# pathwaycom/pathway

Hardware: AMD Instinct MI355X
Metric: events/sec (whole node) on WordCount stream + p50 RAG query latency at fixed QPS (higher is better)
Workload: dtype int64/string-dict; 1 GPU; model=wordcount: stream -> groupby(word).count -> output deltas, global_batch=4000000, seq_len=1, parallelism=dp1 (shard exchange: RCCL all-to-all), vocab=50000, ingest=bytes, emitted_delta_rows=126750000, dict_misses=0

## Files before the change

pathway_amd/ops/__init__.py:

```python

from __future__ import annotations

import contextlib
import ctypes
import os
from typing import Sequence

import torch

_THIS = os.path.dirname(os.path.abspath(__file__))
_LIB_PATH = os.path.join(_THIS, "libpwhip.so")

_lib = None
_load_error: Exception | None = None


def _try_load():
    global _lib, _load_error
    if _lib is not None:
        return _lib
    try:
        if not os.path.exists(_LIB_PATH):
            from pathway_amd.ops import build as _build

# ... 1301 lines not shown
    vals = torch.empty((nq, k), dtype=torch.float32, device=scores.device)
    idx = torch.empty((nq, k), dtype=torch.int64, device=scores.device)
    if nq == 0:
        return vals, idx
    rc = lib.pw_topk(
        ctypes.c_void_p(scores.contiguous().data_ptr()),
        ctypes.c_int64(nq),
        ctypes.c_int64(m),
        ctypes.c_int(k),
        ctypes.c_void_p(vals.data_ptr()),
        ctypes.c_void_p(idx.data_ptr()),
        _stream_ptr(),
    )
    if rc != 0:
        raise RuntimeError(f"pw_topk failed: hip error {rc}")
    return vals, idx


BM25_TILE = 4096


def bm25_score(
    offsets: torch.Tensor,
    pidx: torch.Tensor,
    ptf: torch.Tensor,
    norm: torch.Tensor,
    q_off: torch.Tensor,
    q_term: torch.Tensor,
    q_idf: torch.Tensor,
    k1: float,
    pad_to: int = 1,
) -> torch.Tensor:
    n = norm.shape[0]
    nq = q_off.shape[0] - 1
    assert offsets.dtype == torch.int64 and pidx.dtype == torch.int32
    assert ptf.dtype == torch.float32 and norm.dtype == torch.float32
    assert q_off.dtype == torch.int32 and q_term.dtype == torch.int32
    assert q_idf.dtype == torch.float32
    assert pidx.shape == ptf.shape and q_term.shape == q_idf.shape
    assert nq >= 0 and offsets.shape[0] >= 1
    k1p1 = float(k1) + 1.0
    n_pad = -(-n // pad_to) * pad_to
    if not norm.is_cuda:
        scores = torch.zeros((nq, n_pad), dtype=torch.float32)
        k1p1_t = torch.tensor(k1p1, dtype=torch.float32)
        qo = q_off.tolist()
        for q in range(nq):
            row = scores[q]
            for t in range(qo[q], qo[q + 1]):
                term = int(q_term[t])
                s, e = int(offsets[term]), int(offsets[term + 1])
                d = pidx[s:e].long()
                tf = ptf[s:e]
                row.index_add_(0, d, q_idf[t] * (tf * k1p1_t) / (tf + norm[d]))
        return scores
    lib = require_lib()
    assert BM25_TILE == lib.pw_bm25_tile(), "BM25_TILE out of step with the kernel"
    scores = torch.empty((nq, n_pad), dtype=torch.float32, device=norm.device)
    if n_pad > n:
        scores[:, n:] = 0.0
    rc = lib.pw_bm25_score(
        ctypes.c_void_p(offsets.contiguous().data_ptr()),
        ctypes.c_void_p(pidx.contiguous().data_ptr()),
        ctypes.c_void_p(ptf.contiguous().data_ptr()),
        ctypes.c_void_p(norm.contiguous().data_ptr()),
        ctypes.c_int64(n),
        ctypes.c_void_p(q_off.contiguous().data_ptr()),
        ctypes.c_void_p(q_term.contiguous().data_ptr()),
        ctypes.c_void_p(q_idf.contiguous().data_ptr()),
        ctypes.c_int64(nq),
        ctypes.c_float(k1p1),
        ctypes.c_void_p(scores.data_ptr()),
        ctypes.c_int64(n_pad),
        _stream_ptr(),
    )
    if rc != 0:
        raise RuntimeError(f"pw_bm25_score failed: hip error {rc}")
    return scores


def merge_consolidate_gpu(
    a_words: Sequence[torch.Tensor],
    a_accs: Sequence[torch.Tensor],
    b_words: Sequence[torch.Tensor],
    b_accs: Sequence[torch.Tensor],
    compare_words: int | None = None,
) -> tuple[list[torch.Tensor], list[torch.Tensor], torch.Tensor]:
    lib = require_lib()
    m = a_words[0].shape[0]
    n = b_words[0].shape[0]
    nw = len(a_words)
    nwc = compare_words or nw
    nacc = len(a_accs)
    assert len(b_accs) == nacc and 1 <= nacc <= 8 and 1 <= nwc <= nw <= 4
    device = a_words[0].device
    total_diag = m + n
    nthreads = max(1, (total_diag + 7) // 8)
    counts = torch.empty(nthreads, dtype=torch.int32, device=device)
    wA = [t.contiguous() for t in a_words]
    wB = [t.contiguous() for t in b_words]
    aA = [t.contiguous() for t in a_accs]
    aB = [t.contiguous() for t in b_accs]
    rc = lib.pw_merge_consolidate_count(
        _ptr_arr(wA),
        _ptr_arr(aA),
        _ptr_arr(wB),
        _ptr_arr(aB),
        ctypes.c_int(nw),
        ctypes.c_int(nwc),
        ctypes.c_int(nacc),
        ctypes.c_int64(m),
        ctypes.c_int64(n),
        ctypes.c_void_p(counts.data_ptr()),
        ctypes.c_int64(nthreads),
        _stream_ptr(),
    )
    if rc != 0:
        raise RuntimeError(f"pw_merge_consolidate_count failed: {rc}")
    csum = torch.cumsum(counts.to(torch.int64), 0)
    total = int(csum[-1].item())
    bases = torch.zeros(nthreads, dtype=torch.int64, device=device)
    bases[1:] = csum[:-1]
    out_words = [
        torch.empty(total, dtype=torch.int64, device=device)
        for _ in range(nw)
    ]
    out_accs = [
        torch.empty(total, dtype=torch.int64, device=device)
        for _ in range(nacc)
    ]
    rep = torch.empty(total, dtype=torch.int64, device=device)
    rc = lib.pw_merge_consolidate_emit(
        _ptr_arr(wA),
        _ptr_arr(aA),
        _ptr_arr(wB),
        _ptr_arr(aB),
        ctypes.c_int(nw),
        ctypes.c_int(nwc),
        ctypes.c_int(nacc),
        ctypes.c_int64(m),
        ctypes.c_int64(n),
        ctypes.c_void_p(bases.data_ptr()),
        ctypes.c_int64(nthreads),
        _ptr_arr(out_words),
        _ptr_arr(out_accs),
        ctypes.c_void_p(rep.data_ptr()),
        _stream_ptr(),
    )
    if rc != 0:
        raise RuntimeError(f"pw_merge_consolidate_emit failed: {rc}")
    return out_words, out_accs, rep


def group_update_gpu(
    a_words: Sequence[torch.Tensor],
    a_accs: Sequence[torch.Tensor],
    b_words: Sequence[torch.Tensor],
    b_accs: Sequence[torch.Tensor],
    out_slots: Sequence[int],
):
    lib = require_lib()
    m = a_words[0].shape[0]
    n = b_words[0].shape[0]
    nacc = len(a_accs)
    assert len(a_words) == 2 and len(b_words) == 2
    assert len(b_accs) == nacc and 1 <= nacc <= 8
    slots = sorted(set(int(s) for s in out_slots))
    assert all(0 <= s < nacc for s in slots)
    mask = 0
    for s in slots:
        mask |= 1 << s
    device = b_words[0].device
    nthreads = max(1, (m + n + 7) // 8)
    counts = torch.empty(nthreads * 4, dtype=torch.int32, device=device)
    bases = torch.empty(nthreads * 3, dtype=torch.int64, device=device)
    totals = torch.empty(3, dtype=torch.int64, device=device)
    wA = [t.contiguous() for t in a_words]
    wB = [t.contiguous() for t in b_words]
    aA = [t.contiguous() for t in a_accs]
    aB = [t.contiguous() for t in b_accs]
    for t in wA + wB + aA + aB:
        assert t.dtype == torch.int64
    rc = lib.pw_group_update_count(
        _ptr_arr(wA),
        _ptr_arr(aA),
        _ptr_arr(wB),
        _ptr_arr(aB),
        ctypes.c_int(nacc),
        ctypes.c_uint(mask),
        ctypes.c_int64(m),
        ctypes.c_int64(n),
        ctypes.c_void_p(counts.data_ptr()),
        ctypes.c_void_p(bases.data_ptr()),
        ctypes.c_void_p(totals.data_ptr()),
        ctypes.c_int64(nthreads),
        _stream_ptr(),
    )
    if rc != 0:
        raise RuntimeError(f"pw_group_update_count failed: {rc}")
    n_keep, n_ret, n_ins = totals.tolist()
    n_out = n_ret + n_ins

    def i64(k):
        return torch.empty(k, dtype=torch.int64, device=device)

    out_words = [i64(n_keep) for _ in range(2)]
    out_accs = [i64(n_keep) for _ in range(nacc)]
    rep = i64(n_keep)
    keys = torch.empty((n_out, 2), dtype=torch.int64, device=device)
    diffs = i64(n_out)
    vals = {s: i64(n_out) for s in slots}
    src = i64(n_out)
    varr = (ctypes.c_void_p * 8)(
        *[ctypes.c_void_p(vals[s].data_ptr() if s in vals else 0) for s in range(8)]
    )
    rc = lib.pw_group_update_emit(
        _ptr_arr(wA),
        _ptr_arr(aA),
        _ptr_arr(wB),
        _ptr_arr(aB),
        ctypes.c_int(nacc),
        ctypes.c_uint(mask),
        ctypes.c_int64(m),
        ctypes.c_int64(n),
        ctypes.c_void_p(bases.data_ptr()),
        ctypes.c_int64(n_ret),
        ctypes.c_int64(nthreads),
        _ptr_arr(out_words),
        _ptr_arr(out_accs),
        ctypes.c_void_p(rep.data_ptr()),
        ctypes.c_void_p(keys.data_ptr()),
        ctypes.c_void_p(diffs.data_ptr()),
        varr,
        ctypes.c_void_p(src.data_ptr()),
        _stream_ptr(),
    )
    if rc != 0:
        raise RuntimeError(f"pw_group_update_emit failed: {rc}")
    return out_words, out_accs, rep, keys, diffs, [vals[s] for s in slots], src


def radix_sort64_gpu(keys: torch.Tensor) -> tuple[torch.Tensor, torch.Tensor]:
    lib = require_lib()
    n = keys.shape[0]
    device = keys.device
    perm = torch.arange(n, dtype=torch.int64, device=device)
    if n <= 1:
        return keys.clone(), perm
    nblocks = max(1, min(1024, (n + (64 * 64) - 1) // (64 * 64)))
    chunk = (n + nblocks * 64 - 1) // (nblocks * 64)
    ka = torch.empty(n, dtype=torch.int64, device=device)
    kb = torch.empty(n, dtype=torch.int64, device=device)
    pa = perm
    pb = torch.empty(n, dtype=torch.int64, device=device)
    rc = lib.pw_radix_flip(
        ctypes.c_void_p(keys.contiguous().data_ptr()),
        ctypes.c_void_p(ka.data_ptr()),
        ctypes.c_int64(n),
        _stream_ptr(),
    )
    if rc != 0:
        raise RuntimeError(f"pw_radix_flip failed: {rc}")
    counts = torch.empty(256 * nblocks, dtype=torch.int32, device=device)
    for p in range(8):
        shift = p * 8
        rc = lib.pw_radix_count(
            ctypes.c_void_p(ka.data_ptr()),
            ctypes.c_int64(n),
            ctypes.c_int(shift),
            ctypes.c_int64(nblocks),
            ctypes.c_int64(chunk),
            ctypes.c_void_p(counts.data_ptr()),
            _stream_ptr(),
        )
        if rc != 0:
            raise RuntimeError(f"pw_radix_count failed: {rc}")
        csum = torch.cumsum(counts.to(torch.int64), 0)
        bases = torch.zeros_like(csum)
        bases[1:] = csum[:-1]
        rc = lib.pw_radix_scatter(
            ctypes.c_void_p(ka.data_ptr()),
            ctypes.c_void_p(pa.data_ptr()),
            ctypes.c_int64(n),
            ctypes.c_int(shift),
            ctypes.c_int64(nblocks),
            ctypes.c_int64(chunk),
            ctypes.c_void_p(bases.data_ptr()),
            ctypes.c_void_p(kb.data_ptr()),
            ctypes.c_void_p(pb.data_ptr()),
            _stream_ptr(),
        )
        if rc != 0:
            raise RuntimeError(f"pw_radix_scatter failed: {rc}")
        ka, kb = kb, ka
        pa, pb = pb, pa
    out = torch.empty(n, dtype=torch.int64, device=device)
    rc = lib.pw_radix_unflip(
        ctypes.c_void_p(ka.data_ptr()),
        ctypes.c_void_p(out.data_ptr()),
        ctypes.c_int64(n),
        _stream_ptr(),
    )
    if rc != 0:
        raise RuntimeError(f"pw_radix_unflip failed: {rc}")
    return out, pa


def scan_positions_gpu(buf: torch.Tensor, target: int) -> torch.Tensor:
    lib = require_lib()
    n = buf.shape[0]
    device = buf.device
    nblocks = max(1, min(2048, (n + 4095) // 4096))
    counts = torch.empty(nblocks, dtype=torch.int64, device=device)
    rc = lib.pw_scan_positions(
        ctypes.c_void_p(buf.contiguous().data_ptr()),
        ctypes.c_int64(n),
        ctypes.c_int(int(target)),
        ctypes.c_void_p(counts.data_ptr()),
        ctypes.c_int64(nblocks),
        _stream_ptr(),
    )
    if rc != 0:
        raise RuntimeError(f"pw_scan_positions failed: {rc}")
    csum = torch.cumsum(counts, 0)
    total = int(csum[-1].item())
    bases = torch.zeros(nblocks, dtype=torch.int64, device=device)
    bases[1:] = csum[:-1]
    out = torch.empty(total, dtype=torch.int64, device=device)
    rc = lib.pw_scan_emit(
        ctypes.c_void_p(buf.contiguous().data_ptr()),
        ctypes.c_int64(n),
        ctypes.c_int(int(target)),
        ctypes.c_void_p(bases.data_ptr()),
        ctypes.c_int64(nblocks),
        ctypes.c_void_p(out.data_ptr()),
        _stream_ptr(),
    )
    if rc != 0:
        raise RuntimeError(f"pw_scan_emit failed: {rc}")
    return out


def sort_repair_gpu(
    k0_sorted: torch.Tensor,
    k1_sorted: torch.Tensor,
    perm: torch.Tensor,
    passes: int = 4,
) -> None:
    lib = require_lib()
    n = k0_sorted.shape[0]
    if n < 2:
        return
    rc = lib.pw_sort_repair(
        ctypes.c_void_p(k0_sorted.data_ptr()),
        ctypes.c_void_p(k1_sorted.data_ptr()),
        ctypes.c_void_p(perm.data_ptr()),
        ctypes.c_int64(n),
        ctypes.c_int(int(passes)),
        _stream_ptr(),
    )
    if rc != 0:
        raise RuntimeError(f"pw_sort_repair failed: hip error {rc}")


def gather_cols_gpu(idx: torch.Tensor, cols: list) -> list:
    lib = require_lib()
    m = idx.shape[0]
    outs: list = [None] * len(cols)
    fused_pos: list[int] = []
    for i, c in enumerate(cols):
        if c.dim() == 1 and c.element_size() == 8 and c.is_contiguous():
            fused_pos.append(i)
        else:
            outs[i] = c[idx] if c.dim() > 1 else c.index_select(0, idx)
    idx = idx.contiguous()
    for start in range(0, len(fused_pos), 8):
        group = fused_pos[start : start + 8]
        srcs = (ctypes.c_void_p * len(group))()
        dsts = (ctypes.c_void_p * len(group))()
        for k, i in enumerate(group):
# ... 210 lines not shown
```

pathway_amd/ops/csrc/hip/pw_kernels.hip:

```cpp
#include <hip/hip_runtime.h>
#include <stdint.h>
#include <stdio.h>

#include <cstring>
#include <rocprim/rocprim.hpp>

#include "../xxhash_common.h"

#define PW_BLOCK 256
#define PW_MAX_GRID 2048

static inline int pw_grid(int64_t n) {
  int64_t g = (n + PW_BLOCK - 1) / PW_BLOCK;
  if (g > PW_MAX_GRID) g = PW_MAX_GRID;
  if (g < 1) g = 1;
  return (int)g;
}


struct WordPtrs {
  const uint64_t* p[20];
};

template <int W>
// ... 942 lines not shown
__device__ int64_t mc_merge_path(McWords A, int64_t m, McWords B, int64_t n,
                                 int64_t d, int nwc) {
  int64_t lo = d > n ? d - n : 0;
  int64_t hi = d < m ? d : m;
  while (lo < hi) {
    int64_t mid = (lo + hi) >> 1;
    if (mc_le(A, mid, B, d - mid - 1, nwc))
      lo = mid + 1;
    else
      hi = mid;
  }
  return lo;
}

#define PW_MC_CHUNK 8

template <bool WRITE>
__device__ void mc_walk(McWords A, McAcc accA, McWords B, McAcc accB,
                        int nw, int nwc, int nacc, int64_t m, int64_t n,
                        int64_t d0, int64_t d1, int* count_out,
                        int64_t base, McWordsMut O, McAccMut accO,
                        int64_t* rep) {
  int64_t ai = mc_merge_path(A, m, B, n, d0, nwc);
  int64_t bi = d0 - ai;
  int64_t d = d0;
  if (d < d1 && bi < n && ai > 0 &&
      !(ai < m && mc_le(A, ai, B, bi, nwc))) {
    if (mc_eq(A, ai - 1, B, bi, nwc)) {
      ++bi;
      ++d;
    }
  }
  int cnt = 0;
  int64_t w = base;
  while (d < d1) {
    bool take_a = (bi >= n) || (ai < m && mc_le(A, ai, B, bi, nwc));
    if (take_a) {
      bool matched = (bi < n) && mc_eq(A, ai, B, bi, nwc);
      long long wsum = accA.p[0][ai] + (matched ? accB.p[0][bi] : 0ll);
      if (wsum != 0) {
        if (WRITE) {
          for (int k = 0; k < nw; ++k) O.p[k][w] = A.p[k][ai];
          for (int c = 0; c < nacc; ++c)
            accO.p[c][w] =
                accA.p[c][ai] + (matched ? accB.p[c][bi] : 0ll);
          rep[w] = ai;
          ++w;
        }
        ++cnt;
      }
      ++ai;
      ++d;
      if (matched) {
        ++bi;
        ++d;
      }
    } else {
      long long wsum = accB.p[0][bi];
      if (wsum != 0) {
        if (WRITE) {
          for (int k = 0; k < nw; ++k) O.p[k][w] = B.p[k][bi];
          for (int c = 0; c < nacc; ++c) accO.p[c][w] = accB.p[c][bi];
          rep[w] = m + bi;
          ++w;
        }
        ++cnt;
      }
      ++bi;
      ++d;
    }
  }
  if (!WRITE) *count_out = cnt;
}

__global__ void k_mc_count(McWords A, McAcc accA, McWords B, McAcc accB,
                           int nw, int nwc, int nacc, int64_t m, int64_t n,
                           int* thread_counts, int64_t nthreads) {
  int64_t t = (int64_t)blockIdx.x * blockDim.x + threadIdx.x;
  if (t >= nthreads) return;
  int64_t total = m + n;
  int64_t d0 = t * PW_MC_CHUNK;
  int64_t d1 = min(d0 + PW_MC_CHUNK, total);
  McAccMut dummy{};
  McWordsMut wdummy{};
  mc_walk<false>(A, accA, B, accB, nw, nwc, nacc, m, n, d0, d1,
                 &thread_counts[t], 0, wdummy, dummy, nullptr);
}

__global__ void k_mc_emit(McWords A, McAcc accA, McWords B, McAcc accB,
                          int nw, int nwc, int nacc, int64_t m, int64_t n,
                          const int64_t* bases, int64_t nthreads,
                          McWordsMut O, McAccMut accO, int64_t* rep) {
  int64_t t = (int64_t)blockIdx.x * blockDim.x + threadIdx.x;
  if (t >= nthreads) return;
  int64_t total = m + n;
  int64_t d0 = t * PW_MC_CHUNK;
  int64_t d1 = min(d0 + PW_MC_CHUNK, total);
  mc_walk<true>(A, accA, B, accB, nw, nwc, nacc, m, n, d0, d1, nullptr,
                bases[t], O, accO, rep);
}

extern "C" int pw_merge_consolidate_count(
    const void** wordsA, const void** accA, const void** wordsB,
    const void** accB, int nw, int nwc, int nacc, int64_t m, int64_t n,
    void* thread_counts, int64_t nthreads, void* stream) {
  if (nacc > 8 || nacc < 1 || nw > 4 || nwc > nw) return 2;
  McAcc A{}, B{};
  McWords WA{}, WB{};
  for (int c = 0; c < nacc; ++c) {
    A.p[c] = (const long long*)accA[c];
    B.p[c] = (const long long*)accB[c];
  }
  for (int k = 0; k < nw; ++k) {
    WA.p[k] = (const int64_t*)wordsA[k];
    WB.p[k] = (const int64_t*)wordsB[k];
  }
  hipStream_t s = (hipStream_t)stream;
  int64_t blocks = (nthreads + PW_BLOCK - 1) / PW_BLOCK;
  hipLaunchKernelGGL(k_mc_count, dim3((uint32_t)blocks), dim3(PW_BLOCK), 0,
                     s, WA, A, WB, B, nw, nwc, nacc, m, n,
                     (int*)thread_counts, nthreads);
  return (int)hipGetLastError();
}

extern "C" int pw_merge_consolidate_emit(
    const void** wordsA, const void** accA, const void** wordsB,
    const void** accB, int nw, int nwc, int nacc, int64_t m, int64_t n,
    const void* bases, int64_t nthreads, void** out_words, void** accO,
    void* rep, void* stream) {
  if (nacc > 8 || nacc < 1 || nw > 4 || nwc > nw) return 2;
  McAcc A{}, B{};
  McAccMut O{};
  McWords WA{}, WB{};
  McWordsMut WO{};
  for (int c = 0; c < nacc; ++c) {
    A.p[c] = (const long long*)accA[c];
    B.p[c] = (const long long*)accB[c];
    O.p[c] = (long long*)accO[c];
  }
  for (int k = 0; k < nw; ++k) {
    WA.p[k] = (const int64_t*)wordsA[k];
    WB.p[k] = (const int64_t*)wordsB[k];
    WO.p[k] = (int64_t*)out_words[k];
  }
  hipStream_t s = (hipStream_t)stream;
  int64_t blocks = (nthreads + PW_BLOCK - 1) / PW_BLOCK;
  hipLaunchKernelGGL(k_mc_emit, dim3((uint32_t)blocks), dim3(PW_BLOCK), 0,
                     s, WA, A, WB, B, nw, nwc, nacc, m, n,
                     (const int64_t*)bases, nthreads, WO, O, (int64_t*)rep);
  return (int)hipGetLastError();
}


struct GuOut {
  int64_t* words[2];
  long long* accs[8];
  int64_t* rep;
  int64_t* keys;
  int64_t* diffs;
  long long* vals[8];
  int64_t* src;
};

#define PW_GU_KEEP 0
#define PW_GU_RET 1
#define PW_GU_INS 2

template <bool WRITE>
__device__ __forceinline__ void gu_brow(McAcc accA, McWords B, McAcc accB,
                                        int nacc, unsigned out_slots,
                                        int64_t m, bool matched, int64_t ai,
                                        int64_t bi, int* cnt, int64_t* w,
                                        const GuOut& O) {
  long long old0 = matched ? accA.p[0][ai] : 0ll;
  long long new0 = old0 + accB.p[0][bi];
  bool old_p = old0 > 0, new_p = new0 > 0;
  bool same = true;
  for (int c = 0; c < nacc; ++c)
    if (((out_slots >> c) & 1u) && accB.p[c][bi] != 0) same = false;
  bool unchanged = old_p && new_p && same;
  if (old_p && !unchanged) {
    if (WRITE) {
      int64_t r = w[PW_GU_RET]++;
      O.keys[2 * r] = B.p[0][bi];
      O.keys[2 * r + 1] = B.p[1][bi];
      O.diffs[r] = -1;
      for (int c = 0; c < nacc; ++c)
        if ((out_slots >> c) & 1u) O.vals[c][r] = accA.p[c][ai];
      O.src[r] = ai;
    }
    ++cnt[PW_GU_RET];
  }
  if (new_p && !unchanged) {
    if (WRITE) {
      int64_t r = w[PW_GU_INS]++;
      O.keys[2 * r] = B.p[0][bi];
      O.keys[2 * r + 1] = B.p[1][bi];
      O.diffs[r] = 1;
      for (int c = 0; c < nacc; ++c)
        if ((out_slots >> c) & 1u)
          O.vals[c][r] = (matched ? accA.p[c][ai] : 0ll) + accB.p[c][bi];
      O.src[r] = matched ? ai : m + bi;
    }
    ++cnt[PW_GU_INS];
  }
}

template <bool WRITE>
__device__ void gu_walk(McWords A, McAcc accA, McWords B, McAcc accB,
                        int nacc, unsigned out_slots, int64_t m, int64_t n,
                        int64_t d0, int64_t d1, int* cnt, int64_t* w,
                        const GuOut& O) {
  int64_t ai = mc_merge_path(A, m, B, n, d0, 2);
  int64_t bi = d0 - ai;
  int64_t d = d0;
  if (d < d1 && bi < n && ai > 0 &&
      !(ai < m && mc_le(A, ai, B, bi, 2))) {
    if (mc_eq(A, ai - 1, B, bi, 2)) {
      ++bi;
      ++d;
    }
  }
  while (d < d1) {
    bool take_a = (bi >= n) || (ai < m && mc_le(A, ai, B, bi, 2));
    if (take_a) {
      bool matched = (bi < n) && mc_eq(A, ai, B, bi, 2);
      long long wsum = accA.p[0][ai] + (matched ? accB.p[0][bi] : 0ll);
      if (wsum != 0) {
        if (WRITE) {
          int64_t r = w[PW_GU_KEEP]++;
          O.words[0][r] = A.p[0][ai];
          O.words[1][r] = A.p[1][ai];
          for (int c = 0; c < nacc; ++c)
            O.accs[c][r] = accA.p[c][ai] + (matched ? accB.p[c][bi] : 0ll);
          O.rep[r] = ai;
        }
        ++cnt[PW_GU_KEEP];
      }
      if (matched) {
        gu_brow<WRITE>(accA, B, accB, nacc, out_slots, m, true, ai, bi, cnt,
                       w, O);
        ++bi;
        ++d;
      }
      ++ai;
      ++d;
    } else {
      long long wsum = accB.p[0][bi];
      if (wsum != 0) {
        if (WRITE) {
          int64_t r = w[PW_GU_KEEP]++;
          O.words[0][r] = B.p[0][bi];
          O.words[1][r] = B.p[1][bi];
          for (int c = 0; c < nacc; ++c) O.accs[c][r] = accB.p[c][bi];
          O.rep[r] = m + bi;
        }
        ++cnt[PW_GU_KEEP];
      }
      gu_brow<WRITE>(accA, B, accB, nacc, out_slots, m, false, ai, bi, cnt, w,
                     O);
      ++bi;
      ++d;
    }
  }
}

__global__ void k_gu_count(McWords A, McAcc accA, McWords B, McAcc accB,
                           int nacc, unsigned out_slots, int64_t m, int64_t n,
                           int4* thread_counts, int64_t nthreads) {
  int64_t t = (int64_t)blockIdx.x * blockDim.x + threadIdx.x;
  if (t >= nthreads) return;
  int64_t d0 = t * PW_MC_CHUNK;
  int64_t d1 = min(d0 + PW_MC_CHUNK, m + n);
  int cnt[3] = {0, 0, 0};
  GuOut none{};
  gu_walk<false>(A, accA, B, accB, nacc, out_slots, m, n, d0, d1, cnt,
                 nullptr, none);
  thread_counts[t] = make_int4(cnt[0], cnt[1], cnt[2], 0);
}

#define PW_GU_SCAN_THREADS 1024
#define PW_GU_SCAN_ITEMS 4

__global__ __launch_bounds__(PW_GU_SCAN_THREADS) void k_gu_scan(
    const int4* thread_counts, int64_t nthreads, int64_t* bases,
    int64_t* totals) {
  __shared__ int wave_tot[PW_GU_SCAN_THREADS / 64][3];
  const int tid = threadIdx.x;
  const int lane = tid & 63;
  const int wave = tid >> 6;
  long long carry[3] = {0, 0, 0};
  const int64_t tile = (int64_t)PW_GU_SCAN_THREADS * PW_GU_SCAN_ITEMS;
  for (int64_t t0 = 0; t0 < nthreads; t0 += tile) {
    int64_t first = t0 + (int64_t)tid * PW_GU_SCAN_ITEMS;
    int v[PW_GU_SCAN_ITEMS][3];
    int sum[3] = {0, 0, 0};
#pragma unroll
    for (int k = 0; k < PW_GU_SCAN_ITEMS; ++k) {
      int4 c = make_int4(0, 0, 0, 0);
      if (first + k < nthreads) c = thread_counts[first + k];
      v[k][0] = c.x;
      v[k][1] = c.y;
      v[k][2] = c.z;
      sum[0] += c.x;
      sum[1] += c.y;
      sum[2] += c.z;
    }
    int incl[3];
#pragma unroll
    for (int a = 0; a < 3; ++a) {
      int x = sum[a];
      for (int dlt = 1; dlt < 64; dlt <<= 1) {
        int y = __shfl_up(x, dlt, 64);
        if (lane >= dlt) x += y;
      }
      incl[a] = x;
      if (lane == 63) wave_tot[wave][a] = x;
    }
    __syncthreads();
#pragma unroll
    for (int a = 0; a < 3; ++a) {
      int before = 0, all = 0;
      for (int wv = 0; wv < PW_GU_SCAN_THREADS / 64; ++wv) {
        int wt = wave_tot[wv][a];
        if (wv < wave) before += wt;
        all += wt;
      }
      long long run = carry[a] + before + incl[a] - sum[a];
#pragma unroll
      for (int k = 0; k < PW_GU_SCAN_ITEMS; ++k) {
        if (first + k < nthreads) bases[(first + k) * 3 + a] = run;
        run += v[k][a];
      }
      carry[a] += all;
    }
    __syncthreads();
  }
  if (tid < 3) totals[tid] = carry[tid];
}

__global__ void k_gu_emit(McWords A, McAcc accA, McWords B, McAcc accB,
                          int nacc, unsigned out_slots, int64_t m, int64_t n,
                          const int64_t* bases, int64_t n_ret,
                          int64_t nthreads, GuOut O) {
  int64_t t = (int64_t)blockIdx.x * blockDim.x + threadIdx.x;
  if (t >= nthreads) return;
  int64_t d0 = t * PW_MC_CHUNK;
  int64_t d1 = min(d0 + PW_MC_CHUNK, m + n);
  int cnt[3] = {0, 0, 0};
  int64_t w[3] = {bases[t * 3 + PW_GU_KEEP], bases[t * 3 + PW_GU_RET],
                  n_ret + bases[t * 3 + PW_GU_INS]};
  gu_walk<true>(A, accA, B, accB, nacc, out_slots, m, n, d0, d1, cnt, w, O);
}

static void gu_args(const void** wordsA, const void** accA,
                    const void** wordsB, const void** accB, int nacc,
                    McWords* WA, McAcc* A, McWords* WB, McAcc* B) {
  for (int c = 0; c < nacc; ++c) {
    A->p[c] = (const long long*)accA[c];
    B->p[c] = (const long long*)accB[c];
  }
  for (int k = 0; k < 2; ++k) {
    WA->p[k] = (const int64_t*)wordsA[k];
    WB->p[k] = (const int64_t*)wordsB[k];
  }
}

extern "C" int pw_group_update_count(
    const void** wordsA, const void** accA, const void** wordsB,
    const void** accB, int nacc, unsigned out_slots, int64_t m, int64_t n,
    void* thread_counts, void* bases, void* totals, int64_t nthreads,
    void* stream) {
  if (nacc > 8 || nacc < 1 || nthreads < 1) return 2;
  McAcc A{}, B{};
  McWords WA{}, WB{};
  gu_args(wordsA, accA, wordsB, accB, nacc, &WA, &A, &WB, &B);
  hipStream_t s = (hipStream_t)stream;
  int64_t blocks = (nthreads + PW_BLOCK - 1) / PW_BLOCK;
  hipLaunchKernelGGL(k_gu_count, dim3((uint32_t)blocks), dim3(PW_BLOCK), 0, s,
                     WA, A, WB, B, nacc, out_slots, m, n,
                     (int4*)thread_counts, nthreads);
  hipLaunchKernelGGL(k_gu_scan, dim3(1), dim3(PW_GU_SCAN_THREADS), 0, s,
                     (const int4*)thread_counts, nthreads, (int64_t*)bases,
                     (int64_t*)totals);
  return (int)hipGetLastError();
}

extern "C" int pw_group_update_emit(
    const void** wordsA, const void** accA, const void** wordsB,
    const void** accB, int nacc, unsigned out_slots, int64_t m, int64_t n,
    const void* bases, int64_t n_ret, int64_t nthreads, void** out_words,
    void** out_accs, void* rep, void* out_keys, void* out_diffs,
    void** out_vals, void* src, void* stream) {
  if (nacc > 8 || nacc < 1 || nthreads < 1) return 2;
  McAcc A{}, B{};
  McWords WA{}, WB{};
  gu_args(wordsA, accA, wordsB, accB, nacc, &WA, &A, &WB, &B);
  GuOut O{};
  for (int k = 0; k < 2; ++k) O.words[k] = (int64_t*)out_words[k];
  for (int c = 0; c < nacc; ++c) {
    O.accs[c] = (long long*)out_accs[c];
    if ((out_slots >> c) & 1u) O.vals[c] = (long long*)out_vals[c];
  }
  O.rep = (int64_t*)rep;
  O.keys = (int64_t*)out_keys;
  O.diffs = (int64_t*)out_diffs;
  O.src = (int64_t*)src;
  hipStream_t s = (hipStream_t)stream;
  int64_t blocks = (nthreads + PW_BLOCK - 1) / PW_BLOCK;
  hipLaunchKernelGGL(k_gu_emit, dim3((uint32_t)blocks), dim3(PW_BLOCK), 0, s,
                     WA, A, WB, B, nacc, out_slots, m, n,
                     (const int64_t*)bases, n_ret, nthreads, O);
  return (int)hipGetLastError();
}


#define PW_RS_THREADS 64
#define PW_RS_DIGITS 256

__global__ __launch_bounds__(PW_RS_THREADS) void k_rs_flip(
    const int64_t* in, uint64_t* out, int64_t n, int dir) {
  for (int64_t i = (int64_t)blockIdx.x * blockDim.x + threadIdx.x; i < n;
       i += (int64_t)gridDim.x * blockDim.x)
    out[i] = (uint64_t)in[i] ^ 0x8000000000000000ull;
}

__global__ __launch_bounds__(PW_RS_THREADS) void k_rs_count(
    const uint64_t* keys, int64_t n, int shift, int64_t chunk,
    int* block_digit_counts ,
    int64_t nblocks) {
  __shared__ int cnt[PW_RS_THREADS][PW_RS_DIGITS];
  int lane = threadIdx.x;
  for (int d = 0; d < PW_RS_DIGITS; ++d) cnt[lane][d] = 0;
  int64_t start = ((int64_t)blockIdx.x * PW_RS_THREADS + lane) * chunk;
  int64_t end = min(start + chunk, n);
  for (int64_t i = start; i < end; ++i) {
    int d = (int)((keys[i] >> shift) & 0xFF);
    ++cnt[lane][d];
  }
  __syncthreads();
  for (int d = lane; d < PW_RS_DIGITS; d += PW_RS_THREADS) {
    int s = 0;
    for (int t = 0; t < PW_RS_THREADS; ++t) s += cnt[t][d];
    block_digit_counts[(int64_t)d * nblocks + blockIdx.x] = s;
  }
}

__global__ __launch_bounds__(PW_RS_THREADS) void k_rs_scatter(
    const uint64_t* keys, const int64_t* payload, int64_t n, int shift,
    int64_t chunk, const long long* bases ,
    int64_t nblocks, uint64_t* out_keys, int64_t* out_payload) {
  __shared__ long long lane_base[PW_RS_THREADS][PW_RS_DIGITS];
  int lane = threadIdx.x;
  for (int d = 0; d < PW_RS_DIGITS; ++d) lane_base[lane][d] = 0;
  int64_t start = ((int64_t)blockIdx.x * PW_RS_THREADS + lane) * chunk;
  int64_t end = min(start + chunk, n);
  for (int64_t i = start; i < end; ++i) {
    int d = (int)((keys[i] >> shift) & 0xFF);
    ++lane_base[lane][d];
  }
  __syncthreads();
  for (int d = lane; d < PW_RS_DIGITS; d += PW_RS_THREADS) {
    long long run = bases[(int64_t)d * nblocks + blockIdx.x];
    for (int t = 0; t < PW_RS_THREADS; ++t) {
      long long c = lane_base[t][d];
      lane_base[t][d] = run;
      run += c;
    }
  }
  __syncthreads();
  for (int64_t i = start; i < end; ++i) {
    int d = (int)((keys[i] >> shift) & 0xFF);
    long long p = lane_base[lane][d]++;
    out_keys[p] = keys[i];
    out_payload[p] = payload[i];
  }
}

__global__ __launch_bounds__(PW_RS_THREADS) void k_rs_unflip(
    const uint64_t* in, int64_t* out, int64_t n) {
  for (int64_t i = (int64_t)blockIdx.x * blockDim.x + threadIdx.x; i < n;
       i += (int64_t)gridDim.x * blockDim.x)
    out[i] = (int64_t)(in[i] ^ 0x8000000000000000ull);
}

extern "C" int pw_radix_flip(const void* in, void* out, int64_t n,
                             void* stream) {
  hipStream_t s = (hipStream_t)stream;
  int64_t blocks = min((int64_t)2048, (n + PW_RS_THREADS - 1) / PW_RS_THREADS);
  if (blocks < 1) blocks = 1;
  hipLaunchKernelGGL(k_rs_flip, dim3((uint32_t)blocks), dim3(PW_RS_THREADS),
                     0, s, (const int64_t*)in, (uint64_t*)out, n, 0);
  return (int)hipGetLastError();
}

extern "C" int pw_radix_unflip(const void* in, void* out, int64_t n,
                               void* stream) {
  hipStream_t s = (hipStream_t)stream;
  int64_t blocks = min((int64_t)2048, (n + PW_RS_THREADS - 1) / PW_RS_THREADS);
  if (blocks < 1) blocks = 1;
  hipLaunchKernelGGL(k_rs_unflip, dim3((uint32_t)blocks),
                     dim3(PW_RS_THREADS), 0, s, (const uint64_t*)in,
                     (int64_t*)out, n);
  return (int)hipGetLastError();
}

extern "C" int pw_radix_count(const void* keys, int64_t n, int shift,
                              int64_t nblocks, int64_t chunk, void* counts,
                              void* stream) {
  hipStream_t s = (hipStream_t)stream;
  hipLaunchKernelGGL(k_rs_count, dim3((uint32_t)nblocks),
                     dim3(PW_RS_THREADS), 0, s, (const uint64_t*)keys, n,
                     shift, chunk, (int*)counts, nblocks);
  return (int)hipGetLastError();
}

extern "C" int pw_radix_scatter(const void* keys, const void* payload,
                                int64_t n, int shift, int64_t nblocks,
                                int64_t chunk, const void* bases,
                                void* out_keys, void* out_payload,
                                void* stream) {
  hipStream_t s = (hipStream_t)stream;
  hipLaunchKernelGGL(k_rs_scatter, dim3((uint32_t)nblocks),
                     dim3(PW_RS_THREADS), 0, s, (const uint64_t*)keys,
                     (const int64_t*)payload, n, shift, chunk,
                     (const long long*)bases, nblocks, (uint64_t*)out_keys,
                     (int64_t*)out_payload);
  return (int)hipGetLastError();
}


__device__ __forceinline__ unsigned pw_granule_mask(const uint8_t* buf,
                                                    int64_t g, int64_t end,
                                                    uint8_t t, bool aligned) {
  unsigned m = 0;
  if (aligned && g + 16 <= end) {
    uint4 v = *(const uint4*)(buf + g);
    const uint32_t w[4] = {v.x, v.y, v.z, v.w};
#pragma unroll
    for (int q = 0; q < 4; ++q)
#pragma unroll
      for (int j = 0; j < 4; ++j)
        if (((w[q] >> (8 * j)) & 0xFFu) == t) m |= 1u << (4 * q + j);
  } else {
    for (int j = 0; j < 16 && g + j < end; ++j)
      if (buf[g + j] == t) m |= 1u << j;
  }
  return m;
}

__global__ void k_scan_count(const uint8_t* buf, int64_t n, int target,
                             int64_t chunk, long long* block_counts) {
  __shared__ int cnt;
  if (threadIdx.x == 0) cnt = 0;
  __syncthreads();
  int64_t start = (int64_t)blockIdx.x * chunk;
  int64_t end = min(start + chunk, n);
  const bool aligned = (((size_t)buf & 15) == 0);
  int local = 0;
  for (int64_t tile = start; tile < end; tile += (int64_t)blockDim.x * 16) {
    int64_t g = tile + (int64_t)threadIdx.x * 16;
    if (g < end)
      local += __popc(pw_granule_mask(buf, g, end, (uint8_t)target, aligned));
  }
  atomicAdd(&cnt, local);
// ... 2522 lines not shown
```

Before: 3.938 billion events/s.

## Tile group-update merge into LDS-staged workgroups with wave-level merge path

Replaces the per-thread global merge-path search in the group-update count and emit kernels with per-tile workgroups. Each workgroup finds its tile edges with a wave-cooperative ballot search and stages the keys and first accumulator of both inputs into padded LDS. Per-thread walks then read from LDS, and a packed intra-tile scan records each thread's output offsets and start position, so emit skips the search entirely. The aim is to cut redundant global binary searches and scattered global loads, and to shrink the global scan to one entry per tile. In exchange it adds LDS pressure, 16-bit packed counts that assume small tiles, and more complex edge handling.

Result: slower. 3.833 billion events/s (-2.7%).

```diff
diff --git a/pathway_amd/ops/__init__.py b/pathway_amd/ops/__init__.py
--- a/pathway_amd/ops/__init__.py
+++ b/pathway_amd/ops/__init__.py
@@ -1477,6 +1477,21 @@
     return out_words, out_accs, rep
 
 
+GROUP_UPDATE_TILE = 2048
+
+_gu_threads: int | None = None
+
+
+def _gu_geometry(lib) -> int:
+    global _gu_threads
+    if _gu_threads is None:
+        lib.pw_gu_tile.restype = ctypes.c_int64
+        lib.pw_gu_threads.restype = ctypes.c_int64
+        assert int(lib.pw_gu_tile()) == GROUP_UPDATE_TILE
+        _gu_threads = int(lib.pw_gu_threads())
+    return _gu_threads
+
+
 def group_update_gpu(
     a_words: Sequence[torch.Tensor],
     a_accs: Sequence[torch.Tensor],
@@ -1496,16 +1511,24 @@
     for s in slots:
         mask |= 1 << s
     device = b_words[0].device
-    nthreads = max(1, (m + n + 7) // 8)
-    counts = torch.empty(nthreads * 4, dtype=torch.int32, device=device)
-    bases = torch.empty(nthreads * 3, dtype=torch.int64, device=device)
-    totals = torch.empty(3, dtype=torch.int64, device=device)
+    threads = _gu_geometry(lib)
+    ntiles = max(1, (m + n + GROUP_UPDATE_TILE - 1) // GROUP_UPDATE_TILE)
+    scratch = torch.empty(ntiles * (7 + threads) + 3, dtype=torch.int64, device=device)
+    counts = scratch[: 2 * ntiles]
+    bases = scratch[2 * ntiles : 5 * ntiles]
+    edges = scratch[5 * ntiles : 7 * ntiles]
+    offs = scratch[7 * ntiles : 7 * ntiles + ntiles * threads]
+    totals = scratch[7 * ntiles + ntiles * threads :]
     wA = [t.contiguous() for t in a_words]
     wB = [t.contiguous() for t in b_words]
     aA = [t.contiguous() for t in a_accs]
     aB = [t.contiguous() for t in b_accs]
     for t in wA + wB + aA + aB:
         assert t.dtype == torch.int64
+    for t in wA + aA:
+        assert t.shape[0] == m
+    for t in wB + aB:
+        assert t.shape[0] == n
     rc = lib.pw_group_update_count(
         _ptr_arr(wA),
         _ptr_arr(aA),
@@ -1516,9 +1539,11 @@
         ctypes.c_int64(m),
         ctypes.c_int64(n),
         ctypes.c_void_p(counts.data_ptr()),
+        ctypes.c_void_p(edges.data_ptr()),
+        ctypes.c_void_p(offs.data_ptr()),
         ctypes.c_void_p(bases.data_ptr()),
         ctypes.c_void_p(totals.data_ptr()),
-        ctypes.c_int64(nthreads),
+        ctypes.c_int64(ntiles),
         _stream_ptr(),
     )
     if rc != 0:
@@ -1549,8 +1574,10 @@
         ctypes.c_int64(m),
         ctypes.c_int64(n),
         ctypes.c_void_p(bases.data_ptr()),
+        ctypes.c_void_p(edges.data_ptr()),
+        ctypes.c_void_p(offs.data_ptr()),
         ctypes.c_int64(n_ret),
-        ctypes.c_int64(nthreads),
+        ctypes.c_int64(ntiles),
         _ptr_arr(out_words),
         _ptr_arr(out_accs),
         ctypes.c_void_p(rep.data_ptr()),
diff --git a/pathway_amd/ops/csrc/hip/pw_kernels.hip b/pathway_amd/ops/csrc/hip/pw_kernels.hip
--- a/pathway_amd/ops/csrc/hip/pw_kernels.hip
+++ b/pathway_amd/ops/csrc/hip/pw_kernels.hip
@@ -1118,6 +1118,26 @@
 }
 
 
+#ifndef PW_GU_TILE
+#define PW_GU_TILE 2048
+#endif
+#define PW_GU_CHUNK 8
+#define PW_GU_THREADS (PW_GU_TILE / PW_GU_CHUNK)
+#define PW_GU_ROWS (PW_GU_TILE + 3)
+#define PW_GU_SLOT(i) ((i) + ((i) >> 3))
+#define PW_GU_SLOTS (PW_GU_SLOT(PW_GU_ROWS) + 1)
+
+static_assert(PW_GU_TILE % (64 * PW_GU_CHUNK) == 0, "whole waves per tile");
+static_assert(PW_GU_THREADS <= 1024, "one workgroup per tile");
+static_assert(PW_GU_TILE < 65536, "16-bit offsets inside a tile");
+static_assert(PW_GU_THREADS >= 128, "one wave per tile edge");
+static_assert(PW_GU_SLOTS * 24 <= 64 * 1024, "static LDS limit");
+
+#define PW_GU_EACH(i, count) \
+  _Pragma("unroll") for (int i = 0; i < 8; ++i) if (i < (count))
+#define PW_GU_FROM1(i, count) \
+  _Pragma("unroll") for (int i = 1; i < 8; ++i) if (i < (count))
+
 struct GuOut {
   int64_t* words[2];
   long long* accs[8];
@@ -1132,26 +1152,126 @@
 #define PW_GU_RET 1
 #define PW_GU_INS 2
 
+struct GuTile {
+  const longlong2* key;
+  const long long* wgt;
+  int64_t as0, bs0;
+  int na;
+  __device__ __forceinline__ longlong2 a(int64_t ai) const {
+    return key[PW_GU_SLOT((int)(ai - as0))];
+  }
+  __device__ __forceinline__ longlong2 b(int64_t bi) const {
+    return key[PW_GU_SLOT(na + (int)(bi - bs0))];
+  }
+  __device__ __forceinline__ long long wa(int64_t ai) const {
+    return wgt[PW_GU_SLOT((int)(ai - as0))];
+  }
+  __device__ __forceinline__ long long wb(int64_t bi) const {
+    return wgt[PW_GU_SLOT(na + (int)(bi - bs0))];
+  }
+};
+
+__device__ __forceinline__ bool gu_le(longlong2 x, longlong2 y) {
+  return x.x != y.x ? x.x < y.x : x.y <= y.y;
+}
+
+__device__ __forceinline__ bool gu_eq(longlong2 x, longlong2 y) {
+  return x.x == y.x && x.y == y.y;
+}
+
+__device__ __forceinline__ GuTile gu_stage(McWords A, McAcc accA, McWords B,
+                                           McAcc accB, int64_t m, int64_t n,
+                                           int64_t a_lo, int64_t a_hi,
+                                           int64_t b_lo, int64_t b_hi,
+                                           longlong2* s_key, long long* s_wgt) {
+  GuTile V;
+  V.key = s_key;
+  V.wgt = s_wgt;
+  V.as0 = a_lo > 0 ? a_lo - 1 : 0;
+  V.bs0 = b_lo;
+  V.na = (int)(min(a_hi + 1, m) - V.as0);
+  int nb = (int)(min(b_hi + 1, n) - V.bs0);
+  for (int i = threadIdx.x; i < V.na + nb; i += PW_GU_THREADS) {
+    longlong2 k;
+    long long w;
+    if (i < V.na) {
+      k.x = A.p[0][V.as0 + i];
+      k.y = A.p[1][V.as0 + i];
+      w = accA.p[0][V.as0 + i];
+    } else {
+      int64_t j = V.bs0 + (i - V.na);
+      k.x = B.p[0][j];
+      k.y = B.p[1][j];
+      w = accB.p[0][j];
+    }
+    s_key[PW_GU_SLOT(i)] = k;
+    s_wgt[PW_GU_SLOT(i)] = w;
+  }
+  __syncthreads();
+  return V;
+}
+
+__device__ __forceinline__ int64_t gu_tile_path(const GuTile& V, int64_t d,
+                                                int64_t a_lo, int64_t a_hi,
+                                                int64_t b_lo, int64_t b_hi) {
+  int64_t lo = max(a_lo, d - b_hi);
+  int64_t hi = min(a_hi, d - b_lo);
+  while (lo < hi) {
+    int64_t mid = (lo + hi) >> 1;
+    if (gu_le(V.a(mid), V.b(d - mid - 1)))
+      lo = mid + 1;
+    else
+      hi = mid;
+  }
+  return lo;
+}
+
+__device__ int64_t gu_wave_path(McWords A, int64_t m, McWords B, int64_t n,
+                                int64_t d) {
+  const int lane = threadIdx.x & 63;
+  int64_t lo = d > n ? d - n : 0;
+  int64_t hi = d < m ? d : m;
+  while (lo < hi) {
+    const int64_t len = hi - lo;
+    const bool last = len <= 64;
+    const int64_t mid = last ? lo + lane : lo + (len * lane) / 64;
+    bool le = false;
+    if (mid < hi) {
+      const int64_t j = d - mid - 1;
+      const int64_t a0 = A.p[0][mid], b0 = B.p[0][j];
+      le = a0 != b0 ? a0 < b0 : A.p[1][mid] <= B.p[1][j];
+    }
+    const int t = __popcll(__ballot(le));
+    if (last) return lo + t;
+    const int64_t below = t > 0 ? lo + (len * (t - 1)) / 64 + 1 : lo;
+    if (t < 64) hi = lo + (len * t) / 64;
+    lo = below;
+  }
+  return lo;
+}
+
 template <bool WRITE>
-__device__ __forceinline__ void gu_brow(McAcc accA, McWords B, McAcc accB,
-                                        int nacc, unsigned out_slots,
-                                        int64_t m, bool matched, int64_t ai,
-                                        int64_t bi, int* cnt, int64_t* w,
+__device__ __forceinline__ void gu_brow(McAcc accA, McAcc accB, longlong2 kb,
+                                        long long wa, long long wb, int nacc,
+                                        unsigned out_slots, int64_t m,
+                                        bool matched, int64_t ai, int64_t bi,
+                                        int* cnt, int64_t* w,
                                         const GuOut& O) {
-  long long old0 = matched ? accA.p[0][ai] : 0ll;
-  long long new0 = old0 + accB.p[0][bi];
+  long long old0 = matched ? wa : 0ll;
+  long long new0 = old0 + wb;
   bool old_p = old0 > 0, new_p = new0 > 0;
-  bool same = true;
-  for (int c = 0; c < nacc; ++c)
+  bool same = !((out_slots & 1u) && wb != 0);
+  PW_GU_FROM1(c, nacc)
     if (((out_slots >> c) & 1u) && accB.p[c][bi] != 0) same = false;
   bool unchanged = old_p && new_p && same;
   if (old_p && !unchanged) {
     if (WRITE) {
       int64_t r = w[PW_GU_RET]++;
-      O.keys[2 * r] = B.p[0][bi];
-      O.keys[2 * r + 1] = B.p[1][bi];
+      O.keys[2 * r] = kb.x;
+      O.keys[2 * r + 1] = kb.y;
       O.diffs[r] = -1;
-      for (int c = 0; c < nacc; ++c)
+      if (out_slots & 1u) O.vals[0][r] = old0;
+      PW_GU_FROM1(c, nacc)
         if ((out_slots >> c) & 1u) O.vals[c][r] = accA.p[c][ai];
       O.src[r] = ai;
     }
@@ -1160,10 +1280,11 @@
   if (new_p && !unchanged) {
     if (WRITE) {
       int64_t r = w[PW_GU_INS]++;
-      O.keys[2 * r] = B.p[0][bi];
-      O.keys[2 * r + 1] = B.p[1][bi];
+      O.keys[2 * r] = kb.x;
+      O.keys[2 * r + 1] = kb.y;
       O.diffs[r] = 1;
-      for (int c = 0; c < nacc; ++c)
+      if (out_slots & 1u) O.vals[0][r] = new0;
+      PW_GU_FROM1(c, nacc)
         if ((out_slots >> c) & 1u)
           O.vals[c][r] = (matched ? accA.p[c][ai] : 0ll) + accB.p[c][bi];
       O.src[r] = matched ? ai : m + bi;
@@ -1173,76 +1294,133 @@
 }
 
 template <bool WRITE>
-__device__ void gu_walk(McWords A, McAcc accA, McWords B, McAcc accB,
-                        int nacc, unsigned out_slots, int64_t m, int64_t n,
-                        int64_t d0, int64_t d1, int* cnt, int64_t* w,
-                        const GuOut& O) {
-  int64_t ai = mc_merge_path(A, m, B, n, d0, 2);
+__device__ __forceinline__ void gu_walk(const GuTile& V, McAcc accA,
+                                        McAcc accB, int nacc,
+                                        unsigned out_slots, int64_t m,
+                                        int64_t n, int64_t ai, int64_t d0,
+                                        int64_t d1, int* cnt, int64_t* w,
+                                        const GuOut& O) {
   int64_t bi = d0 - ai;
   int64_t d = d0;
-  if (d < d1 && bi < n && ai > 0 &&
-      !(ai < m && mc_le(A, ai, B, bi, 2))) {
-    if (mc_eq(A, ai - 1, B, bi, 2)) {
+  if (d < d1 && bi < n && ai > 0 && !(ai < m && gu_le(V.a(ai), V.b(bi)))) {
+    if (gu_eq(V.a(ai - 1), V.b(bi))) {
       ++bi;
       ++d;
     }
   }
   while (d < d1) {
-    bool take_a = (bi >= n) || (ai < m && mc_le(A, ai, B, bi, 2));
+    longlong2 ka = make_longlong2(0, 0), kb = make_longlong2(0, 0);
+    long long wa = 0, wb = 0;
+    if (ai < m) {
+      ka = V.a(ai);
+      wa = V.wa(ai);
+    }
+    if (bi < n) {
+      kb = V.b(bi);
+      wb = V.wb(bi);
+    }
+    bool take_a = (bi >= n) || (ai < m && gu_le(ka, kb));
     if (take_a) {
-      bool matched = (bi < n) && mc_eq(A, ai, B, bi, 2);
-      long long wsum = accA.p[0][ai] + (matched ? accB.p[0][bi] : 0ll);
+      bool matched = (bi < n) && gu_eq(ka, kb);
+      long long wsum = wa + (matched ? wb : 0ll);
       if (wsum != 0) {
         if (WRITE) {
           int64_t r = w[PW_GU_KEEP]++;
-          O.words[0][r] = A.p[0][ai];
-          O.words[1][r] = A.p[1][ai];
-          for (int c = 0; c < nacc; ++c)
+          O.words[0][r] = ka.x;
+          O.words[1][r] = ka.y;
+          O.accs[0][r] = wsum;
+          PW_GU_FROM1(c, nacc)
             O.accs[c][r] = accA.p[c][ai] + (matched ? accB.p[c][bi] : 0ll);
           O.rep[r] = ai;
         }
         ++cnt[PW_GU_KEEP];
       }
       if (matched) {
-        gu_brow<WRITE>(accA, B, accB, nacc, out_slots, m, true, ai, bi, cnt,
-                       w, O);
+        gu_brow<WRITE>(accA, accB, kb, wa, wb, nacc, out_slots, m, true, ai,
+                       bi, cnt, w, O);
         ++bi;
         ++d;
       }
       ++ai;
       ++d;
     } else {
-      long long wsum = accB.p[0][bi];
-      if (wsum != 0) {
+      if (wb != 0) {
         if (WRITE) {
           int64_t r = w[PW_GU_KEEP]++;
-          O.words[0][r] = B.p[0][bi];
-          O.words[1][r] = B.p[1][bi];
-          for (int c = 0; c < nacc; ++c) O.accs[c][r] = accB.p[c][bi];
+          O.words[0][r] = kb.x;
+          O.words[1][r] = kb.y;
+          O.accs[0][r] = wb;
+          PW_GU_FROM1(c, nacc) O.accs[c][r] = accB.p[c][bi];
           O.rep[r] = m + bi;
         }
         ++cnt[PW_GU_KEEP];
       }
-      gu_brow<WRITE>(accA, B, accB, nacc, out_slots, m, false, ai, bi, cnt, w,
-                     O);
+      gu_brow<WRITE>(accA, accB, kb, wa, wb, nacc, out_slots, m, false, ai,
+                     bi, cnt, w, O);
       ++bi;
       ++d;
     }
   }
 }
 
-__global__ void k_gu_count(McWords A, McAcc accA, McWords B, McAcc accB,
-                           int nacc, unsigned out_slots, int64_t m, int64_t n,
-                           int4* thread_counts, int64_t nthreads) {
-  int64_t t = (int64_t)blockIdx.x * blockDim.x + threadIdx.x;
-  if (t >= nthreads) return;
-  int64_t d0 = t * PW_MC_CHUNK;
-  int64_t d1 = min(d0 + PW_MC_CHUNK, m + n);
+__global__ __launch_bounds__(PW_GU_THREADS) void k_gu_tile_count(
+    McWords A, McAcc accA, McWords B, McAcc accB, int nacc,
+    unsigned out_slots, int64_t m, int64_t n, int4* tile_counts,
+    int64_t* tile_edges, unsigned long long* thread_offs) {
+  __shared__ longlong2 s_key[PW_GU_SLOTS];
+  __shared__ long long s_wgt[PW_GU_SLOTS];
+  __shared__ int64_t s_edge[2];
+  __shared__ unsigned long long s_wave[PW_GU_THREADS / 64];
+  const int tid = threadIdx.x;
+  const int64_t tile = blockIdx.x;
+  const int64_t D0 = tile * PW_GU_TILE;
+  const int64_t D1 = min(D0 + PW_GU_TILE, m + n);
+  if (tid < 128) {
+    const int64_t e = gu_wave_path(A, m, B, n, tid < 64 ? D0 : D1);
+    if ((tid & 63) == 0) s_edge[tid >> 6] = e;
+  }
+  __syncthreads();
+  const int64_t a_lo = s_edge[0], a_hi = s_edge[1];
+  const int64_t b_lo = D0 - a_lo, b_hi = D1 - a_hi;
+  GuTile V = gu_stage(A, accA, B, accB, m, n, a_lo, a_hi, b_lo, b_hi, s_key,
+                      s_wgt);
+
+  const int64_t d0 = D0 + (int64_t)tid * PW_GU_CHUNK;
+  const int64_t d1 = min(d0 + PW_GU_CHUNK, D1);
   int cnt[3] = {0, 0, 0};
-  GuOut none{};
-  gu_walk<false>(A, accA, B, accB, nacc, out_slots, m, n, d0, d1, cnt,
-                 nullptr, none);
-  thread_counts[t] = make_int4(cnt[0], cnt[1], cnt[2], 0);
+  int64_t ai = a_lo;
+  if (d0 < d1) {
+    ai = gu_tile_path(V, d0, a_lo, a_hi, b_lo, b_hi);
+    GuOut none{};
+    gu_walk<false>(V, accA, accB, nacc, out_slots, m, n, ai, d0, d1, cnt,
+                   nullptr, none);
+  }
+  const unsigned long long mine = (unsigned long long)cnt[PW_GU_KEEP] |
+                                  ((unsigned long long)cnt[PW_GU_RET] << 16) |
+                                  ((unsigned long long)cnt[PW_GU_INS] << 32);
+  const int lane = tid & 63, wave = tid >> 6;
+  unsigned long long incl = mine;
+  for (int dlt = 1; dlt < 64; dlt <<= 1) {
+    unsigned long long y = __shfl_up(incl, dlt, 64);
+    if (lane >= dlt) incl += y;
+  }
+  if (lane == 63) s_wave[wave] = incl;
+  __syncthreads();
+  unsigned long long before = 0, all = 0;
+  for (int wv = 0; wv < PW_GU_THREADS / 64; ++wv) {
+    unsigned long long wt = s_wave[wv];
+    if (wv < wave) before += wt;
+    all += wt;
+  }
+  thread_offs[tile * PW_GU_THREADS + tid] =
+      (before + incl - mine) | ((unsigned long long)(ai - a_lo) << 48);
+  if (tid == 0) {
+    tile_counts[tile] =
+        make_int4((int)(all & 0xffff), (int)((all >> 16) & 0xffff),
+                  (int)((all >> 32) & 0xffff), 0);
+    tile_edges[2 * tile] = a_lo;
+    tile_edges[2 * tile + 1] = a_hi;
+  }
 }
 
 #define PW_GU_SCAN_THREADS 1024
@@ -1305,18 +1483,40 @@
   if (tid < 3) totals[tid] = carry[tid];
 }
 
-__global__ void k_gu_emit(McWords A, McAcc accA, McWords B, McAcc accB,
-                          int nacc, unsigned out_slots, int64_t m, int64_t n,
-                          const int64_t* bases, int64_t n_ret,
-                          int64_t nthreads, GuOut O) {
-  int64_t t = (int64_t)blockIdx.x * blockDim.x + threadIdx.x;
-  if (t >= nthreads) return;
-  int64_t d0 = t * PW_MC_CHUNK;
-  int64_t d1 = min(d0 + PW_MC_CHUNK, m + n);
+__global__ __launch_bounds__(PW_GU_THREADS) void k_gu_tile_emit(
+    McWords A, McAcc accA, McWords B, McAcc accB, int nacc,
+    unsigned out_slots, int64_t m, int64_t n, const int64_t* bases,
+    const int64_t* tile_edges, const unsigned long long* thread_offs,
+    int64_t n_ret, GuOut O) {
+  __shared__ longlong2 s_key[PW_GU_SLOTS];
+  __shared__ long long s_wgt[PW_GU_SLOTS];
+  const int tid = threadIdx.x;
+  const int64_t tile = blockIdx.x;
+  const int64_t D0 = tile * PW_GU_TILE;
+  const int64_t D1 = min(D0 + PW_GU_TILE, m + n);
+  const int64_t a_lo = tile_edges[2 * tile], a_hi = tile_edges[2 * tile + 1];
+  GuTile V = gu_stage(A, accA, B, accB, m, n, a_lo, a_hi, D0 - a_lo,
+                      D1 - a_hi, s_key, s_wgt);
+
+  const int64_t d0 = D0 + (int64_t)tid * PW_GU_CHUNK;
+  const int64_t d1 = min(d0 + PW_GU_CHUNK, D1);
+  if (d0 >= d1) return;
+  const unsigned long long off = thread_offs[tile * PW_GU_THREADS + tid];
   int cnt[3] = {0, 0, 0};
-  int64_t w[3] = {bases[t * 3 + PW_GU_KEEP], bases[t * 3 + PW_GU_RET],
-                  n_ret + bases[t * 3 + PW_GU_INS]};
-  gu_walk<true>(A, accA, B, accB, nacc, out_slots, m, n, d0, d1, cnt, w, O);
+  int64_t w[3] = {
+      bases[tile * 3 + PW_GU_KEEP] + (int64_t)(off & 0xffff),
+      bases[tile * 3 + PW_GU_RET] + (int64_t)((off >> 16) & 0xffff),
+      n_ret + bases[tile * 3 + PW_GU_INS] + (int64_t)((off >> 32) & 0xffff)};
+  gu_walk<true>(V, accA, accB, nacc, out_slots, m, n,
+                a_lo + (int64_t)(off >> 48), d0, d1, cnt, w, O);
+}
+
+extern "C" int64_t pw_gu_tile() { return PW_GU_TILE; }
+extern "C" int64_t pw_gu_threads() { return PW_GU_THREADS; }
+
+static int64_t gu_ntiles(int64_t m, int64_t n) {
+  int64_t t = (m + n + PW_GU_TILE - 1) / PW_GU_TILE;
+  return t < 1 ? 1 : t;
 }
 
 static void gu_args(const void** wordsA, const void** accA,
@@ -1335,19 +1535,21 @@
 extern "C" int pw_group_update_count(
     const void** wordsA, const void** accA, const void** wordsB,
     const void** accB, int nacc, unsigned out_slots, int64_t m, int64_t n,
-    void* thread_counts, void* bases, void* totals, int64_t nthreads,
-    void* stream) {
-  if (nacc > 8 || nacc < 1 || nthreads < 1) return 2;
+    void* tile_counts, void* tile_edges, void* thread_offs, void* bases,
+    void* totals, int64_t ntiles, void* stream) {
+  if (nacc > 8 || nacc < 1 || m < 0 || n < 0) return 2;
+  if (ntiles != gu_ntiles(m, n)) return 2;
+  if (((uintptr_t)tile_counts & 15) != 0) return 2;
   McAcc A{}, B{};
   McWords WA{}, WB{};
   gu_args(wordsA, accA, wordsB, accB, nacc, &WA, &A, &WB, &B);
   hipStream_t s = (hipStream_t)stream;
-  int64_t blocks = (nthreads + PW_BLOCK - 1) / PW_BLOCK;
-  hipLaunchKernelGGL(k_gu_count, dim3((uint32_t)blocks), dim3(PW_BLOCK), 0, s,
-                     WA, A, WB, B, nacc, out_slots, m, n,
-                     (int4*)thread_counts, nthreads);
+  hipLaunchKernelGGL(k_gu_tile_count, dim3((uint32_t)ntiles),
+                     dim3(PW_GU_THREADS), 0, s, WA, A, WB, B, nacc, out_slots,
+                     m, n, (int4*)tile_counts, (int64_t*)tile_edges,
+                     (unsigned long long*)thread_offs);
   hipLaunchKernelGGL(k_gu_scan, dim3(1), dim3(PW_GU_SCAN_THREADS), 0, s,
-                     (const int4*)thread_counts, nthreads, (int64_t*)bases,
+                     (const int4*)tile_counts, ntiles, (int64_t*)bases,
                      (int64_t*)totals);
   return (int)hipGetLastError();
 }
@@ -1355,10 +1557,12 @@
 extern "C" int pw_group_update_emit(
     const void** wordsA, const void** accA, const void** wordsB,
     const void** accB, int nacc, unsigned out_slots, int64_t m, int64_t n,
-    const void* bases, int64_t n_ret, int64_t nthreads, void** out_words,
-    void** out_accs, void* rep, void* out_keys, void* out_diffs,
-    void** out_vals, void* src, void* stream) {
-  if (nacc > 8 || nacc < 1 || nthreads < 1) return 2;
+    const void* bases, const void* tile_edges, const void* thread_offs,
+    int64_t n_ret, int64_t ntiles, void** out_words, void** out_accs,
+    void* rep, void* out_keys, void* out_diffs, void** out_vals, void* src,
+    void* stream) {
+  if (nacc > 8 || nacc < 1 || m < 0 || n < 0) return 2;
+  if (ntiles != gu_ntiles(m, n)) return 2;
   McAcc A{}, B{};
   McWords WA{}, WB{};
   gu_args(wordsA, accA, wordsB, accB, nacc, &WA, &A, &WB, &B);
@@ -1373,10 +1577,10 @@
   O.diffs = (int64_t*)out_diffs;
   O.src = (int64_t*)src;
   hipStream_t s = (hipStream_t)stream;
-  int64_t blocks = (nthreads + PW_BLOCK - 1) / PW_BLOCK;
-  hipLaunchKernelGGL(k_gu_emit, dim3((uint32_t)blocks), dim3(PW_BLOCK), 0, s,
-                     WA, A, WB, B, nacc, out_slots, m, n,
-                     (const int64_t*)bases, n_ret, nthreads, O);
+  hipLaunchKernelGGL(k_gu_tile_emit, dim3((uint32_t)ntiles),
+                     dim3(PW_GU_THREADS), 0, s, WA, A, WB, B, nacc, out_slots,
+                     m, n, (const int64_t*)bases, (const int64_t*)tile_edges,
+                     (const unsigned long long*)thread_offs, n_ret, O);
   return (int)hipGetLastError();
 }
 
diff --git a/profiles/group_update_bench.py b/profiles/group_update_bench.py
--- /dev/null
+++ b/profiles/group_update_bench.py
@@ -0,0 +1,92 @@
+
+from __future__ import annotations
+
+import argparse
+import json
+import statistics
+import time
+
+import torch
+
+from pathway_amd import ops
+
+CALLS = 30
+WARMUP = 5
+
+
+def timed(name: str, fn, rnd: int, **extra) -> None:
+    for _ in range(WARMUP):
+        fn()
+    ms = []
+    for _ in range(CALLS):
+        torch.cuda.synchronize()
+        t0 = time.perf_counter()
+        fn()
+        torch.cuda.synchronize()
+        ms.append((time.perf_counter() - t0) * 1e3)
+    print(json.dumps({
+        "op": name,
+        "round": rnd,
+        "median_ms": round(statistics.median(ms), 4),
+        "max_minus_min_ms": round(max(ms) - min(ms), 4),
+        "min_ms": round(min(ms), 4),
+        "calls": CALLS,
+        **extra,
+    }), flush=True)
+
+
+def side(keys: torch.Tensor, nacc: int, g, weight_lo: int):
+    keys = torch.sort(keys).values
+    words = [keys >> 20, keys & ((1 << 20) - 1)]
+    accs = [torch.randint(weight_lo, 4, keys.shape, device=keys.device, generator=g)]
+    accs += [
+        torch.randint(-3, 4, keys.shape, device=keys.device, generator=g)
+        for _ in range(nacc - 1)
+    ]
+    return words, accs
+
+
+def main() -> None:
+    ap = argparse.ArgumentParser()
+    ap.add_argument("--rounds", type=int, default=2)
+    args = ap.parse_args()
+
+    dev = torch.device("cuda:0")
+    g = torch.Generator(device=dev).manual_seed(1)
+    n = 50_000
+    space = torch.randperm(1 << 24, device=dev, generator=g).to(torch.int64)
+    z = torch.zeros(0, dtype=torch.int64, device=dev)
+
+    aw, aa = side(space[:n], 1, g, 1)
+    bw, ba = side(space[:n], 1, g, 1)
+    ca = torch.randint(0, n, (n,), device=dev, generator=g)
+    cb = torch.randint(0, n, (n,), device=dev, generator=g)
+
+    def flagship():
+        r = ops.group_update_gpu(aw, aa, bw, ba, [0])
+        both = torch.cat([ca, cb])
+        return r + ([both.index_select(0, r[2])], [both.index_select(0, r[6])])
+
+    big = 2_000_000
+    gw, ga = side(space[:big], 1, g, 1)
+    hw, ha = side(space[:big][torch.randperm(big, device=dev, generator=g)[:n]], 1, g, 1)
+    fw, fa = side(space[:n], 1, g, 1)
+    dw, da = side(space[n : 2 * n], 8, g, 1)
+    ew, ea = side(space[2 * n : 3 * n], 8, g, -3)
+
+    jobs = [
+        ("flagship", flagship, dict(m=n, n=n, nacc=1)),
+        ("big_state", lambda: ops.group_update_gpu(gw, ga, hw, ha, [0]),
+         dict(m=big, n=n, nacc=1)),
+        ("first", lambda: ops.group_update_gpu([z, z], [z], fw, fa, [0]),
+         dict(m=0, n=n, nacc=1)),
+        ("disjoint8", lambda: ops.group_update_gpu(dw, da, ew, ea, list(range(8))),
+         dict(m=n, n=n, nacc=8)),
+    ]
+    for rnd in range(args.rounds):
+        for name, fn, extra in jobs:
+            timed(name, fn, rnd, **extra)
+
+
+if __name__ == "__main__":
+    main()
```
